# C-H-Chien/Trifocal_Pose_Estimation_using_Improved_GPUHC

Measured on AMD Instinct MI355X. Metric: HC paths/sec (312 tracks x RANSAC samples), higher is better.
Workload: dtype f32

## Files before the change

trifocal_pose_estimation_using_improved_gpuhc_amd/csrc/hc_kernels.hip:

```cpp
#include "hc_layout.hpp"
#include "hc_prep.hpp"
#include "hc_components.hpp"
#include "hc_ring.hpp"
#include "hc_score.hpp"
#include "hc_track.hpp"
#include "hc_p2c.hpp"
#include "../../include/hc_trifocal_testing.h"
#include "../../include/p2c/hc_trifocal_p2c.h"
#include "../../include/lu/hc_lu_testing.h"
#include "../../include/adaptive/hc_trifocal_adaptive.h"

#include <atomic>
#include <climits>
#include <cstdlib>
#include <cstring>
#include <map>
#include <mutex>
#include <utility>

namespace hc {

thread_local hipError_t g_last_hip_error = hipSuccess;
static inline hcStatus launch_status(hcStatus on_fail) {
    const hipError_t e = hipGetLastError();
// ... 242 lines not shown
        if (e == hipSuccess) e = hipMemcpyAsync(&h_bad, bad, sizeof(unsigned), hipMemcpyDeviceToHost, s);
        if (e == hipSuccess) e = hipStreamSynchronize(s);
        (void)hipFree(bad);
        if (e != hipSuccess) {
            g_last_hip_error = e;
            return HC_ERROR_LAUNCH;
        }
        if (h_bad != 0u) return HC_ERROR_INVALID_VALUE;
    }
    const int per = 2 * WAVES_PER_WG;
    hipLaunchKernelGGL((k_cgesv_variant<M.lat, M.strct, M.entchk, M.fuse>), dim3((n + per - 1) / per), dim3(WG_THREADS), 0, s,
                       n, (const cf *)A, (const cf *)b, (cf *)x);
    return launch_status(HC_ERROR_LAUNCH);
}

}

extern "C" {
#ifdef HC_DIAG_PHASES
int hc_diag_phases(unsigned long long *out, int reset) { return hc::diag_read(hc::g_diag_phase, out, reset); }
#endif
#ifdef HC_DIAG_LUWORK
int hc_diag_luwork(unsigned long long *out, int reset) { return hc::diag_read(hc::g_diag_luwork, out, reset); }
#endif
#ifdef HC_DIAG_LIVE
int hc_diag_live(unsigned long long *out, int reset) { return hc::diag_read(hc::g_diag_live, out, reset); }
#endif
#ifdef HC_DIAG_TIMES
int hc_diag_span(unsigned long long *out, int reset) {
    static const unsigned long long init[4] = {~0ull, 0ull, 0ull, 0ull};
    return hc::diag_read(hc::g_diag_span, out, reset, &init);
}
#endif
#ifdef HC_DIAG_UTIL
int hc_diag_util(unsigned long long *out, int reset) { return hc::diag_read(hc::g_diag_util, out, reset); }
#endif

size_t hc_trifocal_workspace_size(void) { return hc::ws_bytes_needed(); }

size_t hc_trifocal_workspace_size_for(int sub_ransac_iters) {
    return hc_trifocal_workspace_size_for_steps(sub_ransac_iters, 80);
}

size_t hc_trifocal_workspace_size_for_steps(int sub_ransac_iters, int max_steps) {
    return hc::slice_layout(sub_ransac_iters > 0 ? (long long)sub_ransac_iters * hc::NTRK : 0, max_steps).total;
}

hcStatus hc_trifocal_2op1p_30x30_track(const hcTrackArgs *args, void *workspace, size_t workspace_bytes,
                                       hcStream stream) {
    return hc::launch_track(args, {hc::TrackMode::Track}, workspace, workspace_bytes, stream);
}

hcStatus hc_trifocal_2op1p_30x30_track_abort(const hcTrackArgs *args, const hcAbortArgs *abort_args,
                                             void *workspace, size_t workspace_bytes, hcStream stream) {
    return hc::launch_track(args, {hc::TrackMode::Abort, abort_args}, workspace, workspace_bytes, stream);
}

hcStatus hc_trifocal_2op1p_30x30_track_abort_grouped(const hcTrackArgs *args, const hcGroupedAbortArgs *g,
                                                     void *workspace, size_t workspace_bytes, hcStream stream) {
    if (!g) return HC_ERROR_INVALID_VALUE;
    return hc::launch_track(args, {hc::TrackMode::GroupedAbort, nullptr, g}, workspace, workspace_bytes, stream);
}

hcStatus hc_trifocal_2op1p_30x30_track_abort_gated(const hcTrackArgs *args, const hcGroupedAbortArgs *g,
                                                   const hcJointGate *gate, void *workspace,
                                                   size_t workspace_bytes, hcStream stream) {
    if (!g || !gate) return HC_ERROR_INVALID_VALUE;
    if (!(gate->min_joint_ratio > 0.0f) || gate->min_joint_ratio > 3.402823466e+38f) return HC_ERROR_INVALID_VALUE;
    return hc::launch_track(args, {hc::TrackMode::GatedAbort, nullptr, g, gate}, workspace, workspace_bytes, stream);
}

hcStatus hc_trifocal_2op1p_30x30_track_ph_codeopt(const hcTrackArgs *args, void *workspace, size_t workspace_bytes,
                                                  hcStream stream) {
    return hc::launch_track(args, {hc::TrackMode::PhCodeopt}, workspace, workspace_bytes, stream);
}

hcStatus hc_trifocal_2op1p_30x30_track_ph(const hcTrackArgs *args, void *workspace, size_t workspace_bytes,
                                          hcStream stream) {
    return hc::launch_track(args, {hc::TrackMode::Ph}, workspace, workspace_bytes, stream);
}

hcStatus hc_trifocal_2op1p_30x30_track_p2c(const hcTrackArgs *args, const hcP2cArgs *p2c, void *workspace,
                                           size_t workspace_bytes, hcStream stream) {
    if (!p2c || !p2c->hx_index || !p2c->ht_index || !p2c->coeffs_hx || !p2c->coeffs_ht) return HC_ERROR_INVALID_VALUE;
    hc::TrackLaunch l{hc::TrackMode::P2c};
    l.p2c = p2c;
    return hc::launch_track(args, l, workspace, workspace_bytes, stream);
}

hcStatus hc_trifocal_workspace_status(const void *workspace) {
    if (!workspace) return HC_ERROR_INVALID_VALUE;
    hc::Workspace h;
    const hcStatus st = hc::read_control(workspace, h);
    if (st != HC_SUCCESS) return st;
    if (h.status == 0u) return HC_SUCCESS;
    return h.status == (unsigned)HC_ERROR_TABLE ? HC_ERROR_TABLE : HC_ERROR_DEVICE;
}

hcStatus hc_trifocal_read_timings(const void *workspace, double *first_found_seconds) {
    if (!workspace || !first_found_seconds) return HC_ERROR_INVALID_VALUE;
    hc::Workspace h;
    const hcStatus st = hc::read_control(workspace, h);
    if (st != HC_SUCCESS) return st;
    *first_found_seconds = (h.t_found && h.t_start) ? (double)(long long)(h.t_found - h.t_start) / hc::wall_clock_hz() : -1.0;
    return HC_SUCCESS;
}

hcStatus hc_trifocal_read_timestamps(const void *workspace, uint64_t *start_ticks, uint64_t *found_ticks,
                                     double *tick_hz) {
    if (!workspace || !start_ticks || !found_ticks || !tick_hz) return HC_ERROR_INVALID_VALUE;
    hc::Workspace h;
    const hcStatus st = hc::read_control(workspace, h);
    if (st != HC_SUCCESS) return st;
    *start_ticks = h.t_start;
    *found_ticks = h.t_found;
    *tick_hz = hc::wall_clock_hz();
    return HC_SUCCESS;
}

hcStatus hc_cgesv_30x30_batched(int n, const hcComplex *A, const hcComplex *b, hcComplex *x, hcStream stream) {
    if (n < 0 || (n > 0 && (!A || !b || !x))) return HC_ERROR_INVALID_VALUE;
    if (n == 0) return HC_SUCCESS;
    (void)hipGetLastError();
    const int per = 2 * hc::WAVES_PER_WG;
    hipLaunchKernelGGL(hc::k_cgesv, dim3((n + per - 1) / per), dim3(hc::WG_THREADS), 0, (hipStream_t)stream, n,
                       (const hc::cf *)A, (const hc::cf *)b, (hc::cf *)x);
    return hc::launch_status(HC_ERROR_LAUNCH);
}

hcStatus hc_cgesv_30x30_variant_batched(int variant, int n, const hcComplex *A, const hcComplex *b, hcComplex *x,
                                        hcStream stream) {
    if (variant < 0 || variant >= HC_LU_VARIANT_COUNT) return HC_ERROR_INVALID_VALUE;
    if (n < 0 || (n > 0 && (!A || !b || !x))) return HC_ERROR_INVALID_VALUE;
    if (n == 0) return HC_SUCCESS;
    hipStream_t s = (hipStream_t)stream;
    (void)hipGetLastError();
    switch (variant) {
    case HC_LU_VARIANT_THROUGHPUT:      return hc::launch_cgesv_variant<false, false, 0, true>(n, A, b, x, s);
    case HC_LU_VARIANT_THROUGHPUT_TWIN: return hc::launch_cgesv_variant<false, false, 0, false>(n, A, b, x, s);
    case HC_LU_VARIANT_ABORT:           return hc::launch_cgesv_variant<true, false, HC_LU_LATB_COLS, true>(n, A, b, x, s);
    case HC_LU_VARIANT_ABORT_TWIN:      return hc::launch_cgesv_variant<true, false, HC_LU_LATB_COLS, false>(n, A, b, x, s);
    case HC_LU_VARIANT_SMALL:           return hc::launch_cgesv_variant<false, false, HC_SMALL_LAT, true>(n, A, b, x, s);
    case HC_LU_VARIANT_SMALL_TWIN:      return hc::launch_cgesv_variant<false, false, HC_SMALL_LAT, false>(n, A, b, x, s);
    case HC_LU_VARIANT_ARCHIVED:        return hc::launch_cgesv_variant<false, true, 0, true>(n, A, b, x, s);
    case HC_LU_VARIANT_ARCHIVED_TWIN:   return hc::launch_cgesv_variant<false, true, 0, false>(n, A, b, x, s);
    }
    return HC_ERROR_INVALID_VALUE;
}

hcStatus hc_cgesv_30x30_struct_batched(int n, const hcComplex *A, const hcComplex *b, hcComplex *x, hcStream stream) {
    return hc_cgesv_30x30_variant_batched(HC_LU_VARIANT_THROUGHPUT, n, A, b, x, stream);
}

hcStatus hc_trifocal_eval_batched(int n, const int32_t *unified_index, const hcComplex *x, const hcComplex *p,
                                  const hcComplex *d, hcComplex *Hx, hcComplex *Ht, hcComplex *H, void *workspace,
                                  size_t workspace_bytes, hcStream stream) {
    if (n < 0 || !unified_index || (n > 0 && (!x || !p || !d || !Hx || !Ht || !H))) return HC_ERROR_INVALID_VALUE;
    if (!workspace || workspace_bytes < hc::ws_bytes_needed()) return HC_ERROR_WORKSPACE;
    if (n == 0) return HC_SUCCESS;
    hipStream_t s = (hipStream_t)stream;
    hc::Workspace *ws = (hc::Workspace *)workspace;
    (void)hipGetLastError();
    hc::PrepArgs pa{unified_index, ws, nullptr, nullptr, nullptr, nullptr, 0u, 0u, 0u};
    hipLaunchKernelGGL(hc::k_prep_tables, dim3(1), dim3(hc::PREP_THREADS), 0, s, pa);
    if (hc::launch_status(HC_ERROR_LAUNCH) != HC_SUCCESS) return HC_ERROR_LAUNCH;
    const int per = 2 * hc::WAVES_PER_WG;
    hipLaunchKernelGGL(hc::k_eval, dim3((n + per - 1) / per), dim3(hc::WG_THREADS), 0, s, n, ws,
                       (const hc::cf *)x, (const hc::cf *)p, (const hc::cf *)d, (hc::cf *)Hx, (hc::cf *)Ht,
                       (hc::cf *)H);
    return hc::launch_status(HC_ERROR_LAUNCH);
}

hcStatus hc_trifocal_p2c_eval_batched(int n, const int32_t *hx_index, const int32_t *ht_index, const hcComplex *x,
                                      const hcComplex *coeffs_hx, const hcComplex *coeffs_ht, const float *t,
                                      hcComplex *Hx, hcComplex *Ht, hcComplex *H, void *workspace,
                                      size_t workspace_bytes, hcStream stream) {
    if (n < 0 || !hx_index || !ht_index || (n > 0 && (!x || !coeffs_hx || !coeffs_ht || !t || !Hx || !Ht || !H)))
        return HC_ERROR_INVALID_VALUE;
    if (!workspace || workspace_bytes < hc::ws_bytes_needed()) return HC_ERROR_WORKSPACE;
    if (n == 0) return HC_SUCCESS;
    hipStream_t s = (hipStream_t)stream;
    hc::Workspace *ws = (hc::Workspace *)workspace;
    (void)hipGetLastError();
    hc::PrepArgs pa{hx_index, ws, nullptr, nullptr, nullptr, nullptr, 0u, 0u, 0u};
    hipLaunchKernelGGL(hc::k_prep_tables_p2c<true>, dim3(1), dim3(hc::PREP_THREADS), 0, s, pa, ht_index);
    if (hc::launch_status(HC_ERROR_LAUNCH) != HC_SUCCESS) return HC_ERROR_LAUNCH;
    const int per = 2 * hc::WAVES_PER_WG;
    hipLaunchKernelGGL(hc::k_eval_p2c<true>, dim3((n + per - 1) / per), dim3(hc::WG_THREADS), 0, s, n, ws,
                       (const hc::cf *)x, (const hc::cf *)coeffs_hx, (const hc::cf *)coeffs_ht, t, (hc::cf *)Hx,
                       (hc::cf *)Ht, (hc::cf *)H);
    return hc::launch_status(HC_ERROR_LAUNCH);
}

const char *hc_last_error_string(void) { return hipGetErrorString(hc::g_last_hip_error); }

static_assert(sizeof(hcIpcHandle) == sizeof(hipIpcMemHandle_t), "hcIpcHandle mirrors hipIpcMemHandle_t");

namespace hc {
static std::mutex g_flag_mu;
static std::map<const void *, int> g_flag_kind;
}

hcStatus hc_shared_flag_create(uint32_t **flag, hcIpcHandle *handle) {
    if (!flag || !handle) return HC_ERROR_INVALID_VALUE;
    static const unsigned kinds[3] = {hipDeviceMallocUncached, hipDeviceMallocFinegrained, hipDeviceMallocDefault};
    hipError_t last = hipSuccess;
    for (int k = 0; k < 3; k++) {
        void *p = nullptr;
        last = (kinds[k] == hipDeviceMallocDefault) ? hipMalloc(&p, 256) : hipExtMallocWithFlags(&p, 256, kinds[k]);
        if (last != hipSuccess) { (void)hipGetLastError(); continue; }
        hipIpcMemHandle_t h;
        if ((last = hipMemset(p, 0, 256)) != hipSuccess || (last = hipDeviceSynchronize()) != hipSuccess ||
            (last = hipIpcGetMemHandle(&h, p)) != hipSuccess) {
            (void)hipGetLastError();
            (void)hipFree(p);
            continue;
        }
        memcpy(handle, &h, sizeof(h));
        *flag = (uint32_t *)p;
        std::lock_guard<std::mutex> g(hc::g_flag_mu);
        hc::g_flag_kind[p] = 2 - k;
        return HC_SUCCESS;
    }
    hc::g_last_hip_error = last;
    return HC_ERROR_DEVICE;
}

int hc_shared_flag_memory_kind(const uint32_t *flag) {
    std::lock_guard<std::mutex> g(hc::g_flag_mu);
    const auto it = hc::g_flag_kind.find(flag);
    return it == hc::g_flag_kind.end() ? -1 : it->second;
}

hcStatus hc_shared_flag_open(const hcIpcHandle *handle, uint32_t **flag) {
    if (!flag || !handle) return HC_ERROR_INVALID_VALUE;
    hipIpcMemHandle_t h;
    memcpy(&h, handle, sizeof(h));
    void *p = nullptr;
    if ((hc::g_last_hip_error = hipIpcOpenMemHandle(&p, h, hipIpcMemLazyEnablePeerAccess)) != hipSuccess)
        return HC_ERROR_DEVICE;
    *flag = (uint32_t *)p;
    return HC_SUCCESS;
}

hcStatus hc_shared_flag_reset(uint32_t *flag, hcStream stream) {
    if (!flag) return HC_ERROR_INVALID_VALUE;
    if ((hc::g_last_hip_error = hipMemsetAsync(flag, 0, sizeof(uint32_t), (hipStream_t)stream)) != hipSuccess)
        return HC_ERROR_LAUNCH;
    return HC_SUCCESS;
}

hcStatus hc_shared_flag_close(uint32_t *flag, int opened) {
    if (!flag) return HC_ERROR_INVALID_VALUE;
    if (!opened) {
        std::lock_guard<std::mutex> g(hc::g_flag_mu);
        hc::g_flag_kind.erase(flag);
    }
    hc::g_last_hip_error = opened ? hipIpcCloseMemHandle(flag) : hipFree(flag);
    return hc::g_last_hip_error == hipSuccess ? HC_SUCCESS : HC_ERROR_DEVICE;
}

int hc_trifocal_abi_version(void) { return HC_TRIFOCAL_ABI_VERSION; }

unsigned hc_lu_struct_pattern(int row) { return row >= 0 && row < hc::NV ? hc::LU_STRUCT_PAT[row] : 0u; }
unsigned hc_lu_candidates(int step) { return step >= 0 && step < hc::NV ? hc::LU_BOUND.cand[step] : 0u; }
int hc_lu_search_span(int step) { return step >= 0 && step < hc::NV ? hc::lu_search_span(step) : -1; }
int hc_lu_step_level(int step) { return step >= 0 && step < hc::NV ? hc::LU_LEVELS.level[step] : -1; }
int hc_lu_group_class(int step, int group) {
    if (step < 0 || step >= hc::NV - 1 || group < 0 || group >= hc::LuChunks::count(step)) return -1;
    return hc::lu_group_class(step, group);
}

hcStatus hc_trifocal_ring_check_test(void *workspace, size_t workspace_bytes, unsigned head, unsigned tail,
                                     unsigned avail, hcStream stream) {
    const hc::SliceLayout area = hc::slice_layout(0, 0);
    if (!workspace || workspace_bytes < area.ring) return HC_ERROR_WORKSPACE;
    hipStream_t s = (hipStream_t)stream;
    unsigned *rq = (unsigned *)((char *)workspace + area.rq);
    const unsigned v[3] = {head, tail, avail};
    const int at[3] = {hc::RQ_HEAD, hc::RQ_TAIL, hc::RQ_AVAIL};
    (void)hipGetLastError();
    for (int i = 0; i < 3; i++)
        if ((hc::g_last_hip_error = hipMemcpyAsync(rq + at[i], &v[i], sizeof(unsigned), hipMemcpyHostToDevice, s)) !=
            hipSuccess)
            return HC_ERROR_LAUNCH;
    if ((hc::g_last_hip_error = hipStreamSynchronize(s)) != hipSuccess) return HC_ERROR_DEVICE;
    hipLaunchKernelGGL(hc::k_ring_check, dim3(1), dim3(64), 0, s, (hc::Workspace *)workspace, (const unsigned *)rq);
    return hc::launch_status(HC_ERROR_LAUNCH);
}

void hc_trifocal_set_ring_test(int delay_ticks) {
    hc::g_ring_test.store(delay_ticks > 0 ? (delay_ticks < HC_RING_TEST_MIN_TICKS ? HC_RING_TEST_MIN_TICKS : delay_ticks)
                                          : 0,
                          std::memory_order_relaxed);
}

void hc_trifocal_set_small_launch(int mode) {
    hc::g_small_launch.store(mode < 0 ? -1 : mode > 0 ? 1 : 0, std::memory_order_relaxed);
}

void hc_trifocal_set_retry_reuse(int on) { hc::g_retry_reuse.store(on ? 1 : 0, std::memory_order_relaxed); }

const char *hc_trifocal_version(void) {
    return "hc_trifocal gfx950 v10.10 (2 paths/wave, structurally sparse LDS-broadcast LU with lean pivot steps fused by level, "
           "one exec region per pivot step for the eligible rows with the column groups through scratch windows, "
           "column groups by structural class (never-fillable groups untested, always-live groups unconditional), "
           "pivot search narrowed to the candidate rows' DPP group "
           "(abort kernel and tracking launches filling at most half of the path slots -- the latter at 3 waves/SIMD, "
           "16 columns per batch: batched latency mode, one LDS round trip per pivot step, every live-able column "
           "group untested), "
           "structure-agnostic twin kernels for other dH/dx structures, readlane back substitution, pipelined evals over "
           "per-slot prefix tables, 5 waves/SIMD, time slicing at step boundaries with least-attained-service "
           "issue priority, a rejected step's retry reuses its first RK4 slope, the throughput kernel's operand "
           "addresses read complete from per-slot tables and its finiteness check made on the dH/dx entries)";
}

}
```

trifocal_pose_estimation_using_improved_gpuhc_amd/csrc/hc_lu.hpp:

```cpp
#pragma once

#include "hc_eval.hpp"
#include "hc_lu_struct.hpp"
#include "hc_lu_diag.hpp"

namespace hc {

typedef float f4v __attribute__((ext_vector_type(4)));

struct alignas(16) LUBuf {
    cf row[32];
};
static_assert(sizeof(LUBuf) == sizeof(SlotLDS::lu), "LUBuf is SlotLDS::lu");
static_assert(offsetof(SlotLDS, lu) % 16 == 0, "SlotLDS::lu must be 16-B aligned");

__device__ __forceinline__ float rcp_rn(float s) {
    const float r0 = __builtin_amdgcn_rcpf(s);
    const float e0 = __builtin_fmaf(-s, r0, 1.0f);
    return __builtin_fmaf(e0, r0, r0);
}
__device__ __forceinline__ bool rcp_fast_bits(int bits) {
    return (uint32_t)(bits - 0x12800000) < (uint32_t)(0x7B800000 - 0x12800000);
}

// ... 133 lines not shown
    using C = LuChunks;
    if constexpr (K < C::count(I)) {
        constexpr int O = LatCols::off(I, K);
        if constexpr (lu_group_class(I, K) != GRP_DEAD && O >= LO && O < HI)
            grp_load<C::start(I, K), C::len(I, K)>(L.row, &u[O - LO]);
        lat_load<I, K + 1, LO, HI>(u, L);
    }
}
template <int I, int K, int LO, int HI, int M>
__device__ __forceinline__ void lat_fma(cf (&rA)[NV], const pf2 &l, const cf (&u)[M]) {
    using C = LuChunks;
    if constexpr (K < C::count(I)) {
        constexpr int O = LatCols::off(I, K);
        if constexpr (lu_group_class(I, K) != GRP_DEAD && O >= LO && O < HI)
            grp_update<C::start(I, K), C::len(I, K)>(rA, l, &u[O - LO]);
        lat_fma<I, K + 1, LO, HI>(rA, l, u);
    }
}
#ifndef HC_LU_LATB_COLS
#define HC_LU_LATB_COLS 8
#endif
template <int I, int LO, int B>
__device__ __forceinline__ void lat_batches(cf (&rA)[NV], const pf2 &l, const LUBuf &L) {
    constexpr int T = LatCols::total(I);
    if constexpr (LO < T) {
        constexpr int HI = LO + B;
        cf u[B + 1];
        lat_load<I, 0, LO, HI>(u, L);
        lat_fma<I, 0, LO, HI>(rA, l, u);
        lat_batches<I, HI, B>(rA, l, L);
    }
}
template <int I, int LAT>
__device__ __forceinline__ void lu_step_batched(cf (&rA)[NV], cf &rB, int &rowid, PivF &my, LUBuf &L, cf *scr,
                                                bool is_piv, pf2 reg_s, pf2 oo_s, bool elig) {
    HC_ISA_MARK_I("lu_store", I);
    cf *wrow = is_piv ? L.row : scr;
    wrow[I] = cmk(reg_s.x, reg_s.y);
    st4(&wrow[30], rB, cmk(__int_as_float(rowid), 0.0f));
    lat_store<I, 0>(rA, wrow);
    wave_lds_sync();
    HC_ISA_MARK_I("lu_rcp", I);
    cf reg, sB0;
    const int piv_pos = lu_read_pivot<I>(L, reg, sB0);
    cf u[LAT + 1];
    lat_load<I, 0, 0, LAT>(u, L);
    rowid = is_piv ? I : (rowid == I ? piv_pos : rowid);
    my.oo.x = is_piv ? oo_s.x : my.oo.x;
    my.oo.y = is_piv ? oo_s.y : my.oo.y;
    asm volatile("" : "+v"(my.oo));
    HC_ISA_MARK_I("lu_update", I);
    if (elig) {
        HC_ISA_MARK_I("lu_mult", I);
        const pf2 lq = pcmul(pf2{rA[I].x, rA[I].y}, pf2{reg.x, reg.y});
        const pf2 lp = {is_piv ? 0.0f : lq.x, is_piv ? 0.0f : lq.y};
        const pf2 bp = pcmsub(pf2{rB.x, rB.y}, lp, pf2{sB0.x, sB0.y});
        rB = cmk(bp.x, bp.y);
        lat_fma<I, 0, 0, LAT>(rA, lp, u);
        lat_batches<I, LAT, LAT>(rA, lp, L);
    }
}

template <int I, int K, bool STRUCT>
__device__ __forceinline__ void lu_group_elig(cf (&rA)[NV], const pf2 &l, uint32_t pmw, uint32_t gb, cf *wrow,
                                              const LUBuf &L HC_LU_WORK_ARG) {
    using C = LuChunks;
    if constexpr (K < C::count(I)) {
        constexpr int J = C::start(I, K), N = C::len(I, K);
        constexpr int CLS = STRUCT ? lu_group_class(I, K) : GRP_TESTED;
        if (CLS != GRP_DEAD && (CLS == GRP_ALWAYS || __builtin_expect(group_live<I, K>(pmw, gb), 1))) {
            grp_store<J, N>(wrow, rA);
            wave_lds_sync();
            HC_LU_WORK(N);
            HC_DIAG_LIVE_HIT(I, K);
            HC_LU_WORK_GROUP();
            cf u[N];
            grp_load<J, N>(L.row, u);
            grp_update<J, N>(rA, l, u);
        }
        __builtin_amdgcn_sched_barrier(0);
        lu_group_elig<I, K + 1, STRUCT>(rA, l, pmw, gb, wrow, L HC_LU_WORK_PASS);
    }
}
template <int I, bool X1, bool STRUCT>
__device__ __forceinline__ void lu_step_tested(cf (&rA)[NV], cf &rB, int &rowid, uint32_t &pat, PivF &my, LUBuf &L,
                                               cf *scr, bool is_piv, int pl0, int pl1, pf2 reg_s, pf2 oo_s,
                                               bool elig HC_LU_WORK_ARG) {
    const uint32_t pp0 = (uint32_t)__builtin_amdgcn_readlane((int)pat, pl0);
    const uint32_t pp1 = (uint32_t)__builtin_amdgcn_readlane((int)pat, pl1);
    const uint32_t pmw = (pp0 | pp1) & (0xFFFFFFFFu << (I + 1));
    const uint32_t gb = group_bits(pmw);
    HC_ISA_MARK_I("lu_store", I);
    cf *wrow;
    if constexpr (X1) {
        wrow = is_piv ? L.row : scr;
        wrow[I] = cmk(reg_s.x, reg_s.y);
        st4(&wrow[30], rB, cmk(__int_as_float(rowid), 0.0f));
    } else if (is_piv) {
        L.row[I] = cmk(reg_s.x, reg_s.y);
        L.row[30] = rB;
        L.row[31].x = __int_as_float(rowid);
    }
    wave_lds_sync();
    HC_ISA_MARK_I("lu_rcp", I);
    cf reg, sB0;
    const int piv_pos = lu_read_pivot<I>(L, reg, sB0);
    if constexpr (X1) {
        rowid = is_piv ? I : (rowid == I ? piv_pos : rowid);
        my.oo.x = is_piv ? oo_s.x : my.oo.x;
        my.oo.y = is_piv ? oo_s.y : my.oo.y;
    } else {
        if (is_piv) rowid = I;
        else if (rowid == I) rowid = piv_pos;
        if (is_piv) my.oo = oo_s;
    }
    asm volatile("" : "+v"(my.oo));
    HC_ISA_MARK_I("lu_update", I);
    if constexpr (!X1) wrow = is_piv ? L.row : scr;
#ifdef HC_DIAG_LUWORK
    lu_work_acc.excl = __builtin_amdgcn_ballot_w64(is_piv);
#endif
    HC_DIAG_LIVE_HIT(I, LIVE_SOLVES);
    if (elig) {
        HC_ISA_MARK_I("lu_mult", I);
        const pf2 lq = pcmul(pf2{rA[I].x, rA[I].y}, pf2{reg.x, reg.y});
        const pf2 lp = {is_piv ? 0.0f : lq.x, is_piv ? 0.0f : lq.y};
        const pf2 bp = pcmsub(pf2{rB.x, rB.y}, lp, pf2{sB0.x, sB0.y});
        rB = cmk(bp.x, bp.y);
        pat |= (uint32_t)__builtin_amdgcn_sbfe((int)pat, I, 1) & pmw;
        lu_group_elig<I, 0, STRUCT>(rA, lp, pmw, gb, wrow, L HC_LU_WORK_PASS);
    }
}

template <int I, int K>
__device__ __forceinline__ void lu_group_dense(cf (&rA)[NV], const pf2 &l, LUBuf &L, bool is_piv,
                                               bool below HC_LU_WORK_ARG) {
    using C = LuChunks;
    if constexpr (K < C::count(I)) {
        constexpr int J = C::start(I, K), N = C::len(I, K);
        if (is_piv) grp_store<J, N>(L.row, rA);
        wave_lds_sync();
        if (below) {
            HC_LU_WORK(N);
            HC_LU_WORK_GROUP();
            cf u[N];
            grp_load<J, N>(L.row, u);
            grp_update<J, N>(rA, l, u);
        }
        __builtin_amdgcn_sched_barrier(0);
        lu_group_dense<I, K + 1>(rA, l, L, is_piv, below HC_LU_WORK_PASS);
    }
}
template <int I>
__device__ __forceinline__ void lu_step_dense(cf (&rA)[NV], cf &rB, int &rowid, PivF &my, LUBuf &L, bool is_piv,
                                              pf2 reg_s, pf2 oo_s, bool elig HC_LU_WORK_ARG) {
    HC_ISA_MARK_I("lu_store", I);
    if (is_piv) {
        L.row[I] = cmk(reg_s.x, reg_s.y);
        L.row[30] = rB;
        L.row[31].x = __int_as_float(rowid);
    }
    wave_lds_sync();
    HC_ISA_MARK_I("lu_rcp", I);
    cf reg, sB0;
    const int piv_pos = lu_read_pivot<I>(L, reg, sB0);
    if (is_piv) rowid = I;
    else if (rowid == I) rowid = piv_pos;
    if (is_piv) my.oo = oo_s;
    asm volatile("" : "+v"(my.oo));
    const bool below = elig && !is_piv;
    pf2 lp = {0.0f, 0.0f};
    if (below) {
        HC_ISA_MARK_I("lu_mult", I);
        lp = pcmul(pf2{rA[I].x, rA[I].y}, pf2{reg.x, reg.y});
        const pf2 bp = pcmsub(pf2{rB.x, rB.y}, lp, pf2{sB0.x, sB0.y});
        rB = cmk(bp.x, bp.y);
    }
    HC_ISA_MARK_I("lu_update", I);
    lu_group_dense<I, 0>(rA, lp, L, is_piv, below HC_LU_WORK_PASS);
}

}

#include "hc_lu_levels.hpp"

namespace hc {

template <int I, bool DENSE, int LAT, bool STRUCT>
__device__ __forceinline__ void lu_forward(cf (&rA)[NV], cf &rB, int &rowid, uint32_t &pat, int lane, int r, int hb,
                                           bool row_lane, PivF &my, LUBuf &L, cf *scr, bool &redo,
                                           unsigned long long elig_m HC_LU_WORK_ARG) {
    if constexpr (I < NV) {
        HC_ISA_MARK_I("lu_search", I);
        const float v = __builtin_fabsf(rA[I].x) + __builtin_fabsf(rA[I].y);
        pf2 reg_s, oo_s;
        if constexpr (!DENSE) {
            reg_s = recip_fast(pf2{rA[I].x, rA[I].y}, v, oo_s);
        } else {
            const divf f = cdiv_factors(rA[I]);
            const cf rg = (v == 0.0f) ? cmk(1.0f, 0.0f) : cdiv_apply(cmk(1.0f, 0.0f), f);
            reg_s = pf2{rg.x, rg.y};
            oo_s = pf2{f.o1, f.o2};
        }
        const bool elig = __builtin_amdgcn_inverse_ballot_w64(elig_m);
        bool is_piv;
        float piv_abs;
        int pl0, pl1;
        unsigned long long piv_m;
        constexpr int SPAN = (STRUCT && !DENSE) ? lu_search_span(I) : 4;
        const int key = elig ? __float_as_int(v) : -1;
        const int mx = half_max_int_span<SPAN>(key);
        unsigned long long m = __builtin_amdgcn_ballot_w64(key == mx);
        unsigned long long bad = __builtin_amdgcn_ballot_w64(!rcp_fast_bits(mx));
        if constexpr (SPAN < 4) {
            m = and_halves<LU_BOUND.cand[I]>(m);
            bad = and_halves<LU_BOUND.cand[I]>(bad);
        }
        const unsigned mlo = (unsigned)m, mhi = (unsigned)(m >> 32);
        constexpr bool TIE = I == 18 || I == 19 || I == 21 || I == 22;
        const bool rare = DENSE || (TIE ? (bad != 0ull) : ((__builtin_popcountll(m) != 2) | (bad != 0ull)));
        if (__builtin_expect(rare, 0)) {
            HC_ISA_MARK_I("lu_rare", I);
#ifdef HC_DIAG_LUWORK
            lu_work_acc.rare++;
            if constexpr (!DENSE) {
                if (lane == 0) atomicAdd(&g_diag_luwork[DIAG_LUWORK_RARE_AT + I], 1ull);
                if (lu_step_fusable(I)) lu_work_acc.rare_fusable = 1ull;
            }
#endif
            const bool isn = v != v;
            const unsigned long long nanb = __builtin_amdgcn_ballot_w64(isn);
            int mx2 = mx;
            unsigned long long m2 = m;
            if constexpr (SPAN < 4) {
                mx2 = half_max_int_p16(key);
                m2 = __builtin_amdgcn_ballot_w64(key == mx2);
            }
            if (__builtin_expect(nanb != 0ull, 0)) {
                const int key2 = (elig && !isn) ? __float_as_int(v) : -1;
                mx2 = half_max_int_p16(key2);
                m2 = __builtin_amdgcn_ballot_w64(key2 == mx2);
            }
            const unsigned long long nanm = nanb & __builtin_amdgcn_ballot_w64(rowid == I);
            const unsigned nlo = (unsigned)nanm, nhi = (unsigned)(nanm >> 32);
            const unsigned mine_m = hb ? (unsigned)(m2 >> 32) : (unsigned)m2, mine_n = hb ? nhi : nlo;
            const int c2 = ((mine_m >> r) & 1u) ? rowid : (1 << 20);
            const int mn = half_min_int_p16(c2);
            const unsigned long long w = __builtin_amdgcn_ballot_w64(row_lane && rowid == mn);
            const unsigned wm = hb ? (unsigned)(w >> 32) : (unsigned)w;
            const int pl = mine_n ? hb + __builtin_ctz(mine_n) : hb + (wm ? __builtin_ctz(wm) : 0);
            is_piv = lane == pl;
            piv_abs = mine_n ? __builtin_nanf("") : __int_as_float(mx2);
            const unsigned long long pm = __builtin_amdgcn_ballot_w64(is_piv);
            piv_m = pm;
            pl0 = __builtin_ctz((unsigned)pm | 0x80000000u);
            pl1 = 32 + __builtin_ctz((unsigned)(pm >> 32) | 0x80000000u);
            if constexpr (!DENSE)
                redo = redo || __builtin_amdgcn_ballot_w64(!rcp_fast_bits(__float_as_int(piv_abs))) != 0ull;
        } else if constexpr (TIE) {
            const int c2 = key == mx ? rowid : (1 << 20);
            const int mn = half_min_int_p16(c2);
            is_piv = key == mx && rowid == mn;
            piv_abs = __int_as_float(mx);
            const unsigned long long w = __builtin_amdgcn_ballot_w64(is_piv);
            piv_m = w;
            pl0 = __builtin_ctz((unsigned)w);
            pl1 = 32 + __builtin_ctz((unsigned)(w >> 32));
        } else {
            is_piv = __builtin_amdgcn_inverse_ballot_w64(m);
            piv_m = m;
            piv_abs = __int_as_float(mx);
            pl0 = __builtin_ctz(mlo);
            pl1 = 32 + __builtin_ctz(mhi);
        }
        HC_ISA_MARK_I("lu_pattern", I);
        if constexpr (DENSE) lu_step_dense<I>(rA, rB, rowid, my, L, is_piv, reg_s, oo_s, elig HC_LU_WORK_PASS);
        else if constexpr (LAT > 0 && STRUCT) lu_step_batched<I, LAT>(rA, rB, rowid, my, L, scr, is_piv, reg_s, oo_s, elig);
        else lu_step_tested<I, (LAT > 0), STRUCT>(rA, rB, rowid, pat, my, L, scr, is_piv, pl0, pl1, reg_s, oo_s,
                                                  elig HC_LU_WORK_PASS);
        lu_forward<I + 1, DENSE, LAT, STRUCT>(rA, rB, rowid, pat, lane, r, hb, row_lane, my, L, scr, redo,
                                              elig_m & ~piv_m HC_LU_WORK_PASS);
    }
}
template <int LV>
__device__ __forceinline__ void lu_forward_fused(cf (&rA)[NV], cf &rB, int &rowid, uint32_t &pat, int lane, int r, int hb,
                                                 bool row_lane, PivF &my, LUBuf &L, cf *scr, bool &redo,
                                                 unsigned long long elig_m HC_LU_WORK_ARG) {
    if constexpr (LV < LU_LEVELS.nlevels) {
        if (!lu_level<LV>(rA, rB, rowid, pat, lane, r, hb, my, scr, elig_m HC_LU_WORK_PASS)) {
#ifdef HC_DIAG_LUWORK
            lu_work_acc.rare++;
            lu_work_acc.rare_fusable = 1ull;
#endif
            redo = true;
            return;
        }
        lu_forward_fused<LV + 1>(rA, rB, rowid, pat, lane, r, hb, row_lane, my, L, scr, redo, elig_m HC_LU_WORK_PASS);
    } else {
        lu_forward<lu_first_unfused_step(), false, 0, true>(rA, rB, rowid, pat, lane, r, hb, row_lane, my, L, scr, redo,
                                                           elig_m HC_LU_WORK_PASS);
    }
}

template <int I>
__device__ __forceinline__ void lu_backward(const cf (&rA)[NV], cf &rB, int rowid, const PivF &my, pf2 &res) {
    if constexpr (I >= 0) {
        HC_ISA_MARK_I("lu_back", I);
        const unsigned long long own = __builtin_amdgcn_ballot_w64(rowid == I);
        const int o0 = __builtin_ctz((unsigned)own);
        const int o1 = 32 + __builtin_ctz((unsigned)(own >> 32));
        const pf2 q = pcdiv_apply(pf2{rB.x, rB.y}, pf2{rA[I].x, rA[I].y}, my);
        const float x0 = __int_as_float(__builtin_amdgcn_readlane(__float_as_int(q.x), o0));
        const float y0 = __int_as_float(__builtin_amdgcn_readlane(__float_as_int(q.y), o0));
        const float x1 = __int_as_float(__builtin_amdgcn_readlane(__float_as_int(q.x), o1));
        const float y1 = __int_as_float(__builtin_amdgcn_readlane(__float_as_int(q.y), o1));
        const pf2 xs0 = {x0, y0}, xs1 = {x1, y1};
        pf2 xv;
        unsigned long long tmp;
        asm volatile("s_nop 1\n\ts_mov_b64 %2, exec\n\tv_mov_b64 %0, %3\n\ts_mov_b32 exec_lo, 0\n\t"
                     "v_mov_b64 %0, %4\n\ts_mov_b32 exec_lo, %5\n\ts_mov_b32 exec_hi, %5\n\t"
                     "v_mov_b64 %1, %0\n\ts_mov_b64 exec, %2"
                     : "=&v"(xv), "+v"(res), "=&s"(tmp) : "s"(xs0), "s"(xs1), "i"(1u << I));
        if constexpr (I > 0) {
            const pf2 w = pcmsub(pf2{rB.x, rB.y}, xv, pf2{rA[I].x, rA[I].y});
            rB = cmk(w.x, w.y);
        }
        lu_backward<I - 1>(rA, rB, rowid, my, res);
    }
}

struct LuMode { int lat; bool strct, entchk, fuse; };
constexpr LuMode lu_mode(bool ABORT, bool ARCH, int LULAT, bool LUS) {
    const bool entchk = !ABORT && !ARCH && LULAT == 0;
    return LuMode{LULAT, LUS, entchk, entchk && LUS};
}

template <bool DENSE, int LAT = 0, bool STRUCT = false, bool ENTCHK = false, bool FUSE = false>
__device__ __forceinline__ cf lu_solve(cf (&rA)[NV], cf rB, int lane, uint32_t pattern, LUBuf &L, cf *scratch,
                                      bool &redo, unsigned long long count_mask = ~0ull, bool ent_bad = false) {
    static_assert(!FUSE || (!DENSE && LAT == 0 && STRUCT && ENTCHK), "the fused levels belong to the throughput tracker's solve");
    (void)count_mask;
    const int r = lane & 31, hb = lane & 32;
    const bool row_lane = r < NV;
    redo = false;
    if constexpr (DENSE) HC_ISA_MARK("lu_dense");
    else HC_ISA_MARK("lu_sparse");
    HC_ISA_MARK("lu_finite");
    if constexpr (!DENSE && ENTCHK) {
        if (__builtin_expect(ent_bad, 0)) {
            redo = true;
            return cmk(0.0f, 0.0f);
        }
    } else if constexpr (!DENSE) {
        pf2 sq = {0.0f, 0.0f};
#pragma unroll
        for (int c = 0; c < NV; c++) {
            const pf2 e = {rA[c].x, rA[c].y};
            asm("v_pk_fma_f32 %0, %1, %1, %0" : "+v"(sq) : "v"(e));
        }
        const bool ok = sq.x + sq.y < __builtin_inff();
        if (__builtin_expect(__builtin_amdgcn_ballot_w64(!ok) != 0ull, 0)) {
            redo = true;
            return cmk(0.0f, 0.0f);
        }
    }
    int rowid = row_lane ? r : 99;
    uint32_t pat = row_lane ? pattern : 0u;
    PivF my{pf2{0.0f, 0.0f}};
#ifdef HC_DIAG_LUWORK
    LuWork lu_work_acc{0ull, count_mask, 0ull, 0ull, 0ull, 0ull};
#endif
    if constexpr (FUSE)
        lu_forward_fused<0>(rA, rB, rowid, pat, lane, r, hb, row_lane, my, L, scratch + 2 * r, redo,
                            __builtin_amdgcn_ballot_w64(row_lane) HC_LU_WORK_PASS);
    else
        lu_forward<0, DENSE, LAT, STRUCT>(rA, rB, rowid, pat, lane, r, hb, row_lane, my, L, scratch + 2 * r, redo,
                                          __builtin_amdgcn_ballot_w64(row_lane) HC_LU_WORK_PASS);
#ifdef HC_DIAG_LUWORK
    const unsigned long long solves = (unsigned long long)__builtin_popcountll(count_mask & __builtin_amdgcn_ballot_w64(row_lane)) / NV;
    if (lane == 0 && !DENSE && !redo) {
        atomicAdd(&g_diag_luwork[0], lu_work_acc.acc);
        atomicAdd(&g_diag_luwork[1], solves);
        atomicAdd(&g_diag_luwork[3], 1ull);
        atomicAdd(&g_diag_luwork[4], lu_work_acc.groups);
        atomicAdd(&g_diag_luwork[5], lu_work_acc.rare);
    }
    if (lane == 0 && DENSE) atomicAdd(&g_diag_luwork[2], solves);
    if (lane == 0 && !DENSE) atomicAdd(&g_diag_luwork[DIAG_LUWORK_RARE_FUSABLE], lu_work_acc.rare_fusable);
#endif
    if constexpr (FUSE) {
        if (__builtin_expect(redo, 0)) return cmk(0.0f, 0.0f);
    }
#ifdef HC_DIAG_PHASES
    if ((lane & 63) == 0 && blockIdx.x < 16384u) g_diag_lu_mid[blockIdx.x * 4 + (threadIdx.x >> 6)] = __builtin_amdgcn_s_memtime();
#endif
    HC_ISA_MARK("lu_back_init");
    pf2 res = {0.0f, 0.0f};
    lu_backward<NV - 1>(rA, rB, rowid, my, res);
    return cmk(res.x, res.y);
}

}
```

trifocal_pose_estimation_using_improved_gpuhc_amd/csrc/hc_lu_levels.hpp:

```cpp
#pragma once

namespace hc {

constexpr int DPP_WAVE_SHL1 = 0x130, DPP_WAVE_SHR1 = 0x138;

template <int LV, int K>
__device__ __forceinline__ void lvl_pick(const cf (&rA)[NV], pf2 &c, uint32_t &bnd, int &cwo) {
    if constexpr (K < lu_level_count(LV)) {
        constexpr int I = lu_level_member(LV, K);
        const bool in = __builtin_amdgcn_inverse_ballot_w64(lu_both(LU_BOUND.cand[I]));
        c.x = in ? rA[I].x : c.x;
        c.y = in ? rA[I].y : c.y;
        bnd = in ? LU_BOUND.s[I] : bnd;
        cwo = in ? LU_CHAIN_WIN0 + 2 * K : cwo;
        lvl_pick<LV, K + 1>(rA, c, bnd, cwo);
    }
}
template <int LV, int K>
__device__ __forceinline__ void lvl_relabel(int &rowid, unsigned long long m, int hb) {
    if constexpr (K < lu_level_count(LV)) {
        constexpr int I = lu_level_member(LV, K);
        const unsigned long long mi = and_halves<LU_BOUND.cand[I]>(m);
        const int p0 = __builtin_amdgcn_readlane(rowid, __builtin_ctz((unsigned)mi));
        const int p1 = __builtin_amdgcn_readlane(rowid, 32 + __builtin_ctz((unsigned)(mi >> 32)));
        const int piv_pos = hb ? p1 : p0;
        const bool is_p = __builtin_amdgcn_inverse_ballot_w64(mi);
        rowid = is_p ? I : (rowid == I ? piv_pos : rowid);
        lvl_relabel<LV, K + 1>(rowid, m, hb);
    }
}
template <int LV, int J>
__device__ __forceinline__ void lvl_groups(cf (&rA)[NV], const pf2 &l, cf *wrow, const cf *cw) {
    if constexpr (J < NV) {
        if constexpr (((LU_LEVELS.cols[LV] >> J) & 3u) != 0u) {
            grp_store<J, 2>(wrow, rA);
            wave_lds_sync();
            cf u[2];
            grp_load<J, 2>(cw, u);
            grp_update<J, 2>(rA, l, u);
            __builtin_amdgcn_sched_barrier(0);
        }
        lvl_groups<LV, J + 2>(rA, l, wrow, cw);
    }
}
template <int LV>
__device__ __forceinline__ bool lu_level(cf (&rA)[NV], cf &rB, int &rowid, uint32_t &pat, int lane, int r, int hb,
                                         PivF &my, cf *scr, unsigned long long &elig_m HC_LU_WORK_ARG) {
    constexpr int CNT = lu_level_count(LV), I0 = lu_level_member(LV, 0);
    constexpr uint32_t ROWS = LU_LEVELS.rows[LV];
    HC_ISA_MARK_I("lu_search", I0);
    pf2 c = {0.0f, 0.0f};
    uint32_t bnd = 0u;
    int cwo = 0;
    lvl_pick<LV, 0>(rA, c, bnd, cwo);
    const float v = __builtin_fabsf(c.x) + __builtin_fabsf(c.y);
    pf2 oo_s;
    const pf2 reg_s = recip_fast(c, v, oo_s);
    const unsigned long long lv_elig = and_halves<ROWS>(elig_m);
    const bool elig = __builtin_amdgcn_inverse_ballot_w64(lv_elig);
    const int key = elig ? __float_as_int(v) : -1;
    int mx;
    {
        const int u1 = dpp_i<DPP_WAVE_SHL1>(key), u2 = dpp_i<DPP_WAVE_SHL1>(u1);
        const int d1 = dpp_i<DPP_WAVE_SHR1>(key), d2 = dpp_i<DPP_WAVE_SHR1>(d1);
        const int a = __builtin_amdgcn_inverse_ballot_w64(lu_both(LU_TRI0 | LU_TRI1)) ? u1 : -1;
        const int b = __builtin_amdgcn_inverse_ballot_w64(lu_both(LU_TRI0)) ? u2 : -1;
        const int e = __builtin_amdgcn_inverse_ballot_w64(lu_both(LU_TRI1 | LU_TRI2)) ? d1 : -1;
        const int f = __builtin_amdgcn_inverse_ballot_w64(lu_both(LU_TRI2)) ? d2 : -1;
        mx = max(max(key, a), max(b, max(e, f)));
    }
    constexpr uint32_t UP9 = lu_partner_rows(LV, 9), DN9 = lu_partner_rows(LV, -9), UP6 = lu_partner_rows(LV, 6),
                       DN6 = lu_partner_rows(LV, -6);
    static_assert((UP9 | DN9 | UP6 | DN6 | lu_partner_rows(LV, 0)) == (1u << NV) - 1u, "partner triples 6 or 9 lanes away");
    if constexpr ((UP9 | DN9 | UP6 | DN6) != 0u) {
        int pl = lane;
        if constexpr (UP9 != 0u) pl = __builtin_amdgcn_inverse_ballot_w64(lu_both(UP9)) ? lane + 9 : pl;
        if constexpr (DN9 != 0u) pl = __builtin_amdgcn_inverse_ballot_w64(lu_both(DN9)) ? lane - 9 : pl;
        if constexpr (UP6 != 0u) pl = __builtin_amdgcn_inverse_ballot_w64(lu_both(UP6)) ? lane + 6 : pl;
        if constexpr (DN6 != 0u) pl = __builtin_amdgcn_inverse_ballot_w64(lu_both(DN6)) ? lane - 6 : pl;
        mx = max(mx, __builtin_amdgcn_ds_bpermute(pl << 2, mx));
    }
    const unsigned long long m = and_halves<ROWS>(__builtin_amdgcn_ballot_w64(key == mx));
    const unsigned long long bad = and_halves<ROWS>(__builtin_amdgcn_ballot_w64(!rcp_fast_bits(mx)));
    if (__builtin_expect((__builtin_popcountll(m) != 2 * CNT) | (bad != 0ull), 0)) return false;
    const bool is_piv = __builtin_amdgcn_inverse_ballot_w64(m);
    HC_ISA_MARK_I("lu_store", I0);
    const cf *cw = scr + (cwo - 2 * r);
    cf *wrow = is_piv ? const_cast<cf *>(cw) : scr;
    st4(&wrow[0], cmk(reg_s.x, reg_s.y), rB);
    wave_lds_sync();
    HC_ISA_MARK_I("lu_rcp", I0);
    cf reg, sB0;
    ld4(&cw[0], reg, sB0);
    if (is_piv) my.oo = oo_s;
    asm volatile("" : "+v"(my.oo));
    lvl_relabel<LV, 0>(rowid, m, hb);
    HC_ISA_MARK_I("lu_update", I0);
#ifdef HC_DIAG_LUWORK
    {
        int pairs = 0;
        for (int j = 0; j < NV; j += 2) pairs += ((LU_LEVELS.cols[LV] >> j) & 3u) != 0u;
        lu_work_acc.acc += 2ull * (unsigned long long)pairs *
                           (unsigned long long)__builtin_popcountll(lv_elig & lu_work_acc.mask & ~m);
        lu_work_acc.groups += (unsigned long long)pairs;
    }
#endif
    if (elig) {
        HC_ISA_MARK_I("lu_mult", I0);
        const pf2 lq = pcmul(c, pf2{reg.x, reg.y});
        const pf2 lp = {is_piv ? 0.0f : lq.x, is_piv ? 0.0f : lq.y};
        const pf2 bp = pcmsub(pf2{rB.x, rB.y}, lp, pf2{sB0.x, sB0.y});
        rB = cmk(bp.x, bp.y);
        pat |= (pat & lu_member_cols(LV)) != 0u ? bnd : 0u;
        lvl_groups<LV, 0>(rA, lp, wrow, cw);
    }
    elig_m &= ~m;
    return true;
}

}
```

trifocal_pose_estimation_using_improved_gpuhc_amd/csrc/hc_lu_struct.hpp:

```cpp
#pragma once

#include <initializer_list>

#include "hc_device.hpp"

namespace hc {

constexpr int LU_CHUNK = 2;

struct LuChunks {
    static constexpr int single(int I) { return ((I + 1) & 1) && (I + 1 < NV) ? 1 : 0; }
    static constexpr int start(int I, int k) { return k < single(I) ? I + 1 : I + 1 + single(I) + (k - single(I)) * LU_CHUNK; }
    static constexpr int len(int I, int k) {
        return k < single(I) ? 1 : ((NV - start(I, k)) < LU_CHUNK ? (NV - start(I, k)) : LU_CHUNK);
    }
    static constexpr int count(int I) { return single(I) + (NV - (I + 1 + single(I)) + LU_CHUNK - 1) / LU_CHUNK; }
    static constexpr uint32_t mask(int I, int k) { return ((1u << len(I, k)) - 1u) << start(I, k); }
};

constexpr uint32_t LU_STRUCT_PAT[NV] = {
    0x7040004u, 0x7080004u, 0x7100004u, 0x7040009u, 0x7080009u, 0x7100009u, 0x7040012u, 0x7080012u,
    0x7100012u, 0x38200020u, 0x38400020u, 0x38800020u, 0x38200041u, 0x38400041u, 0x38800041u, 0x38200082u,
    0x38400082u, 0x38800082u, 0x7003100u, 0x7003100u, 0x7001100u, 0x7018400u, 0x7018400u, 0x7008400u,
    0x38005200u, 0x38005200u, 0x38001200u, 0x38028800u, 0x38028800u, 0x38008800u};
constexpr uint16_t LU_ALWAYS[NV] = {0x2000, 0x1000, 0x1800, 0xc00, 0xc00, 0xd00, 0xc00, 0x600, 0x304, 0x302,
                                    0x184,  0x182,  0x80,   0x60,  0xc0,  0x21,  0x30,  0x30,  0x18,  0,
                                    0,      0,      0,      0,     0,     0,     0,     0,     0,     0};
struct LuBound { uint32_t s[NV], cand[NV]; };
constexpr LuBound lu_struct_bound() {
    LuBound b{};
    uint32_t cur[NV] = {};
    for (int r = 0; r < NV; r++) cur[r] = LU_STRUCT_PAT[r];
    for (int i = 0; i < NV; i++) {
        const uint32_t above = (0xFFFFFFFFu << (i + 1)) & ((1u << NV) - 1u);
        uint32_t u = 0u;
        for (int r = 0; r < NV; r++)
            if ((cur[r] >> i) & 1u) { u |= cur[r]; b.cand[i] |= 1u << r; }
        b.s[i] = u & above;
        for (int r = 0; r < NV; r++)
            if ((cur[r] >> i) & 1u) cur[r] |= u & above;
    }
    return b;
}
constexpr LuBound LU_BOUND = lu_struct_bound();
enum : int { GRP_TESTED = 0, GRP_DEAD = 1, GRP_ALWAYS = 2 };
constexpr int lu_group_class(int I, int K) {
    return (LU_BOUND.s[I] & LuChunks::mask(I, K)) == 0u ? GRP_DEAD
           : ((LU_ALWAYS[I] >> K) & 1u)                     ? GRP_ALWAYS
                                                              : GRP_TESTED;
}
constexpr int lu_search_span(int I) {
    const uint32_t c = LU_BOUND.cand[I];
    if (c == 0u) return 4;
    int lo = 0, hi = 31;
    while (!((c >> lo) & 1u)) lo++;
    while (!((c >> hi) & 1u)) hi--;
    return (lo >> 2) == (hi >> 2) ? 1 : (lo >> 3) == (hi >> 3) ? 2 : (lo >> 4) == (hi >> 4) ? 3 : 4;
}
constexpr bool lu_classes_consistent() {
    for (int i = 0; i < NV - 1; i++)
        for (int k = 0; k < LuChunks::count(i); k++)
            if (((LU_ALWAYS[i] >> k) & 1u) && (LU_BOUND.s[i] & LuChunks::mask(i, k)) == 0u) return false;
    return true;
}
static_assert(lu_classes_consistent(), "LU_ALWAYS names a provably dead group");

constexpr int LU_FUSE_ROWS = 6;
struct LuLevels {
    int level[NV];
    int nlevels;
    uint32_t fused[NV];
    uint32_t rows[NV];
    uint32_t cols[NV];
};
constexpr int lu_popcount(uint32_t x) { int n = 0; for (; x; x &= x - 1u) n++; return n; }
constexpr bool lu_step_fusable(int I) {
    const int n = lu_popcount(LU_BOUND.cand[I]);
    return n > 0 && n <= LU_FUSE_ROWS;
}
constexpr LuLevels lu_struct_levels() {
    LuLevels v{};
    for (int j = 0; j < NV; j++) {
        int l = 0;
        for (int i = 0; i < j; i++)
            if ((LU_BOUND.cand[i] & LU_BOUND.cand[j]) != 0u && v.level[i] + 1 > l) l = v.level[i] + 1;
        v.level[j] = l;
        if (lu_step_fusable(j)) {
            v.fused[l] |= 1u << j;
            v.rows[l] |= LU_BOUND.cand[j];
            v.cols[l] |= LU_BOUND.s[j];
            if (l + 1 > v.nlevels) v.nlevels = l + 1;
        }
    }
    return v;
}
constexpr LuLevels LU_LEVELS = lu_struct_levels();
constexpr bool lu_levels_disjoint() {
    for (int i = 0; i < NV; i++)
        for (int j = i + 1; j < NV; j++)
            if (LU_LEVELS.level[i] == LU_LEVELS.level[j] && (LU_BOUND.cand[i] & LU_BOUND.cand[j]) != 0u) return false;
    return true;
}
constexpr bool lu_levels_ordered() {
    for (int j = 0; j < NV; j++)
        for (int i = 0; i < j; i++)
            if (lu_step_fusable(j) && (LU_BOUND.cand[i] & LU_BOUND.cand[j]) != 0u &&
                !(lu_step_fusable(i) && LU_LEVELS.level[i] < LU_LEVELS.level[j])) return false;
    return true;
}
constexpr uint32_t lu_fused_steps() {
    uint32_t m = 0u;
    for (int l = 0; l < LU_LEVELS.nlevels; l++) m |= LU_LEVELS.fused[l];
    return m;
}
constexpr int lu_first_unfused_step() {
    int i = 0;
    while (i < NV && ((lu_fused_steps() >> i) & 1u)) i++;
    return i;
}
constexpr uint32_t lu_bits(std::initializer_list<int> v) {
    uint32_t m = 0u;
    for (int b : v) m |= 1u << b;
    return m;
}
static_assert(lu_levels_disjoint(), "two steps of one level share a candidate row");
static_assert(lu_levels_ordered(), "a fused step depends on a step outside the lower fused levels");
static_assert(lu_fused_steps() == (1u << 18) - 1u, "the fused levels cover exactly steps 0..17");
static_assert(LU_LEVELS.nlevels == 4 && LU_LEVELS.fused[0] == lu_bits({0, 1, 2, 5, 8, 9, 10, 11}) &&
              LU_LEVELS.fused[1] == lu_bits({3, 4, 12, 15}) && LU_LEVELS.fused[2] == lu_bits({6, 7, 13, 16}) &&
              LU_LEVELS.fused[3] == lu_bits({14, 17}), "the levels of DESIGN.md §3.5");
static_assert(LU_LEVELS.rows[0] == (1u << NV) - 1u && LU_LEVELS.rows[1] == (LU_LEVELS.rows[0] & ~lu_bits({0, 1, 2, 9, 10, 11})) &&
              LU_LEVELS.rows[2] == LU_LEVELS.rows[1] && LU_LEVELS.rows[3] == (0x3FFC0000u & LU_LEVELS.rows[0]),
              "the rows the levels work on");

constexpr int lu_level_count(int lv) { return lu_popcount(LU_LEVELS.fused[lv]); }
constexpr int lu_level_member(int lv, int k) {
    for (int i = 0; i < NV; i++)
        if ((LU_LEVELS.fused[lv] >> i) & 1u) {
            if (k == 0) return i;
            k--;
        }
    return -1;
}
constexpr int lu_max_level_count() {
    int n = 0;
    for (int l = 0; l < LU_LEVELS.nlevels; l++)
        if (lu_level_count(l) > n) n = lu_level_count(l);
    return n;
}
constexpr int lu_partner_off(int lv, int row) {
    for (int k = 0; k < lu_level_count(lv); k++) {
        const uint32_t c = LU_BOUND.cand[lu_level_member(lv, k)];
        if (!((c >> row) & 1u) || lu_popcount(c) <= 3) continue;
        int lo = 0, hi = 31;
        while (!((c >> lo) & 1u)) lo++;
        while (!((c >> hi) & 1u)) hi--;
        return row < lo + 3 ? (hi - 2) - lo : lo - (hi - 2);
    }
    return 0;
}
constexpr uint32_t lu_partner_rows(int lv, int off) {
    uint32_t m = 0u;
    for (int r = 0; r < NV; r++)
        if (lu_partner_off(lv, r) == off) m |= 1u << r;
    return m;
}
constexpr bool lu_chains_are_triples() {
    for (int i = 0; i < NV; i++) {
        if (!lu_step_fusable(i)) continue;
        uint32_t c = LU_BOUND.cand[i], t = 0u;
        for (int q = 0; q < NV; q += 3)
            if (((c >> q) & 7u) == 7u) t |= 7u << q;
        if (t != c) return false;
    }
    return true;
}
static_assert(lu_chains_are_triples(), "a fusable step's candidates are not whole lane triples");
constexpr uint32_t lu_member_cols(int lv) { return LU_LEVELS.fused[lv]; }
constexpr unsigned long long lu_both(uint32_t m) { return (unsigned long long)m | ((unsigned long long)m << 32); }
constexpr uint32_t LU_TRI0 = 0x09249249u, LU_TRI1 = LU_TRI0 << 1, LU_TRI2 = LU_TRI0 << 2;

constexpr int LU_SCRATCH_CF = 2 * 31 + 32;
constexpr int LU_CHAIN_WIN0 = LU_SCRATCH_CF;
constexpr int LU_SCRATCH_FUSED_CF = LU_CHAIN_WIN0 + 2 * (lu_max_level_count() - 1) + 32;

}
```

Before: 1.515 million.

## Back-substitute fused LU positions level by level through LDS

In the throughput kernel's fused LU solve, back substitution for the 18 fused pivot positions now runs per dependency level (4 levels) instead of one serial readlane step per column. Each level solves all its independent positions at once, writes them to the LDS row buffer, and updates the dependent rows after a wave LDS sync. The remaining columns still use the serial readlane path. A NaN ballot afterwards sets redo. New static asserts check that the level ordering is valid for the backward pass. The cost is extra LDS traffic and syncs in place of 18 serial readlane steps.

```diff
diff --git a/trifocal_pose_estimation_using_improved_gpuhc_amd/csrc/hc_kernels.hip b/trifocal_pose_estimation_using_improved_gpuhc_amd/csrc/hc_kernels.hip
--- a/trifocal_pose_estimation_using_improved_gpuhc_amd/csrc/hc_kernels.hip
+++ b/trifocal_pose_estimation_using_improved_gpuhc_amd/csrc/hc_kernels.hip
@@ -568,14 +568,15 @@
 void hc_trifocal_set_retry_reuse(int on) { hc::g_retry_reuse.store(on ? 1 : 0, std::memory_order_relaxed); }
 
 const char *hc_trifocal_version(void) {
-    return "hc_trifocal gfx950 v10.10 (2 paths/wave, structurally sparse LDS-broadcast LU with lean pivot steps fused by level, "
+    return "hc_trifocal gfx950 v10.11 (2 paths/wave, structurally sparse LDS-broadcast LU with lean pivot steps fused by level, "
            "one exec region per pivot step for the eligible rows with the column groups through scratch windows, "
            "column groups by structural class (never-fillable groups untested, always-live groups unconditional), "
            "pivot search narrowed to the candidate rows' DPP group "
            "(abort kernel and tracking launches filling at most half of the path slots -- the latter at 3 waves/SIMD, "
            "16 columns per batch: batched latency mode, one LDS round trip per pivot step, every live-able column "
            "group untested), "
-           "structure-agnostic twin kernels for other dH/dx structures, readlane back substitution, pipelined evals over "
+           "structure-agnostic twin kernels for other dH/dx structures, readlane back substitution (the throughput "
+           "kernel's fused positions level by level through LDS), pipelined evals over "
            "per-slot prefix tables, 5 waves/SIMD, time slicing at step boundaries with least-attained-service "
            "issue priority, a rejected step's retry reuses its first RK4 slope, the throughput kernel's operand "
            "addresses read complete from per-slot tables and its finiteness check made on the dH/dx entries)";
diff --git a/trifocal_pose_estimation_using_improved_gpuhc_amd/csrc/hc_lu.hpp b/trifocal_pose_estimation_using_improved_gpuhc_amd/csrc/hc_lu.hpp
--- a/trifocal_pose_estimation_using_improved_gpuhc_amd/csrc/hc_lu.hpp
+++ b/trifocal_pose_estimation_using_improved_gpuhc_amd/csrc/hc_lu.hpp
@@ -459,9 +459,9 @@
     }
 }
 
-template <int I>
+template <int I, int LAST = 0>
 __device__ __forceinline__ void lu_backward(const cf (&rA)[NV], cf &rB, int rowid, const PivF &my, pf2 &res) {
-    if constexpr (I >= 0) {
+    if constexpr (I >= LAST) {
         HC_ISA_MARK_I("lu_back", I);
         const unsigned long long own = __builtin_amdgcn_ballot_w64(rowid == I);
         const int o0 = __builtin_ctz((unsigned)own);
@@ -482,7 +482,7 @@
             const pf2 w = pcmsub(pf2{rB.x, rB.y}, xv, pf2{rA[I].x, rA[I].y});
             rB = cmk(w.x, w.y);
         }
-        lu_backward<I - 1>(rA, rB, rowid, my, res);
+        lu_backward<I - 1, LAST>(rA, rB, rowid, my, res);
     }
 }
 
@@ -553,7 +553,23 @@
 #endif
     HC_ISA_MARK("lu_back_init");
     pf2 res = {0.0f, 0.0f};
-    lu_backward<NV - 1>(rA, rB, rowid, my, res);
+    if constexpr (FUSE) {
+        lu_backward<NV - 1, lu_first_unfused_step()>(rA, rB, rowid, my, res);
+        lu_backward_fused<LU_LEVELS.nlevels - 1>(rA, rB, rowid, my, L, r, res);
+        const float nf = __builtin_fmaf(res.y, 0.0f, res.x * 0.0f);
+        redo = __builtin_amdgcn_ballot_w64(nf != nf) != 0ull;
+#ifdef HC_DIAG_LUWORK
+        if (lane == 0 && redo) {
+            atomicAdd(&g_diag_luwork[0], 0ull - lu_work_acc.acc);
+            atomicAdd(&g_diag_luwork[1], 0ull - solves);
+            atomicAdd(&g_diag_luwork[3], 0ull - 1ull);
+            atomicAdd(&g_diag_luwork[4], 0ull - lu_work_acc.groups);
+            atomicAdd(&g_diag_luwork[5], 0ull - lu_work_acc.rare);
+        }
+#endif
+    } else {
+        lu_backward<NV - 1>(rA, rB, rowid, my, res);
+    }
     return cmk(res.x, res.y);
 }
 
diff --git a/trifocal_pose_estimation_using_improved_gpuhc_amd/csrc/hc_lu_levels.hpp b/trifocal_pose_estimation_using_improved_gpuhc_amd/csrc/hc_lu_levels.hpp
--- a/trifocal_pose_estimation_using_improved_gpuhc_amd/csrc/hc_lu_levels.hpp
+++ b/trifocal_pose_estimation_using_improved_gpuhc_amd/csrc/hc_lu_levels.hpp
@@ -118,4 +118,51 @@
     return true;
 }
 
+template <int LV, int K>
+__device__ __forceinline__ void lvl_back_pick(const cf (&rA)[NV], pf2 &c, int &mem) {
+    if constexpr (K < lu_level_count(LV)) {
+        constexpr int I = lu_level_member(LV, K);
+        if constexpr (K == 0) {
+            c = pf2{rA[I].x, rA[I].y};
+            mem = I;
+        } else {
+            const bool in = __builtin_amdgcn_inverse_ballot_w64(lu_both(LU_BOUND.cand[I]));
+            c.x = in ? rA[I].x : c.x;
+            c.y = in ? rA[I].y : c.y;
+            mem = in ? I : mem;
+        }
+        lvl_back_pick<LV, K + 1>(rA, c, mem);
+    }
 }
+template <int LV>
+__device__ __forceinline__ void lu_back_level(const cf (&rA)[NV], cf &rB, int rowid, const PivF &my, LUBuf &L) {
+    HC_ISA_MARK_I("lu_back_level", LV);
+    pf2 c;
+    int mem;
+    lvl_back_pick<LV, 0>(rA, c, mem);
+    const pf2 q = pcdiv_apply(pf2{rB.x, rB.y}, c, my);
+    if (rowid == mem) L.row[mem] = cmk(q.x, q.y);
+    wave_lds_sync();
+    if constexpr (LV > 0) {
+        if (__builtin_amdgcn_inverse_ballot_w64(lu_both(LU_LEVELS.rows[LV]))) {
+            const cf x = L.row[mem];
+            const pf2 w = pcmsub(pf2{rB.x, rB.y}, pf2{x.x, x.y}, c);
+            rB = cmk(w.x, w.y);
+        }
+    }
+}
+template <int LV>
+__device__ __forceinline__ void lu_backward_fused(const cf (&rA)[NV], cf &rB, int rowid, const PivF &my, LUBuf &L, int r,
+                                                  pf2 &res) {
+    if constexpr (LV >= 0) {
+        lu_back_level<LV>(rA, rB, rowid, my, L);
+        lu_backward_fused<LV - 1>(rA, rB, rowid, my, L, r, res);
+    } else {
+        if (__builtin_amdgcn_inverse_ballot_w64(lu_both(lu_fused_steps()))) {
+            const cf x = L.row[r];
+            res = pf2{x.x, x.y};
+        }
+    }
+}
+
+}
diff --git a/trifocal_pose_estimation_using_improved_gpuhc_amd/csrc/hc_lu_struct.hpp b/trifocal_pose_estimation_using_improved_gpuhc_amd/csrc/hc_lu_struct.hpp
--- a/trifocal_pose_estimation_using_improved_gpuhc_amd/csrc/hc_lu_struct.hpp
+++ b/trifocal_pose_estimation_using_improved_gpuhc_amd/csrc/hc_lu_struct.hpp
@@ -108,6 +108,25 @@
                 !(lu_step_fusable(i) && LU_LEVELS.level[i] < LU_LEVELS.level[j])) return false;
     return true;
 }
+constexpr bool lu_back_chains_nested() {
+    for (int i = 0; i < NV; i++)
+        for (int j = i + 1; j < NV; j++)
+            if (lu_step_fusable(i) && lu_step_fusable(j) && ((LU_BOUND.s[i] >> j) & 1u) &&
+                !((LU_BOUND.cand[i] & ~LU_BOUND.cand[j]) == 0u && LU_LEVELS.level[i] < LU_LEVELS.level[j])) return false;
+    return true;
+}
+constexpr bool lu_back_order_kept() {
+    for (int r = 0; r < NV; r++) {
+        int last = -1;
+        for (int l = 0; l < NV; l++)
+            for (int i = 0; i < NV; i++)
+                if (lu_step_fusable(i) && LU_LEVELS.level[i] == l && ((LU_BOUND.cand[i] >> r) & 1u)) {
+                    if (i <= last) return false;
+                    last = i;
+                }
+    }
+    return true;
+}
 constexpr uint32_t lu_fused_steps() {
     uint32_t m = 0u;
     for (int l = 0; l < LU_LEVELS.nlevels; l++) m |= LU_LEVELS.fused[l];
@@ -125,6 +144,8 @@
 }
 static_assert(lu_levels_disjoint(), "two steps of one level share a candidate row");
 static_assert(lu_levels_ordered(), "a fused step depends on a step outside the lower fused levels");
+static_assert(lu_back_chains_nested(), "a fused pivot row can hold a fused column outside its chain's ancestors");
+static_assert(lu_back_order_kept(), "a row's ancestors do not rise in column with the level");
 static_assert(lu_fused_steps() == (1u << 18) - 1u, "the fused levels cover exactly steps 0..17");
 static_assert(LU_LEVELS.nlevels == 4 && LU_LEVELS.fused[0] == lu_bits({0, 1, 2, 5, 8, 9, 10, 11}) &&
               LU_LEVELS.fused[1] == lu_bits({3, 4, 12, 15}) && LU_LEVELS.fused[2] == lu_bits({6, 7, 13, 16}) &&
```

Result: faster. 1.606 million, median of 6 (+6.0%).
